# microsoft/Sora

Hardware: AMD Instinct MI355X
Metric: IQ Msamples/s through 802.11a 54 Mbps RX PHY (higher is better)
Workload: dtype int16 IQ / u8 path metrics

## Files before the change

sora_amd/build.py:

```python
import os
import shutil
import subprocess
import sys
from concurrent.futures import ThreadPoolExecutor

HERE = os.path.dirname(os.path.abspath(__file__))
CSRC = os.path.join(HERE, "csrc")
OBJ = os.path.join(HERE, "lib", "obj")
LIB = os.path.join(HERE, "lib", "libsora_hip.so")
SOURCES = ["k_scan.hip", "k_rx.hip", "k_vit16.hip", "k_vitwin.hip", "k_stage.hip", "k_tx.hip", "k_tx11n.hip", "k_tx_ht40.hip", "k_tx11b.hip", "k_mod.hip", "k_mod11n.hip", "k_mod11b.hip",
    "k_mod_ht40.hip", "k_11b.hip", "k_rx11b.hip", "k_11n.hip", "k_11a.hip", "k_rx11n.hip", "k_ht40.hip", "k_ht40_stages.hip", "k_deliver.hip", "sora_hip.cpp", "sora_shard.cpp"]
HEADERS = ["dev_arith.h", "dev_viterbi.h", "dev_vit16.h", "dev_winplan.h", "dev_vitwin.h", "dev_11n.h", "dev_ht40.h", "dev_pilot11a.h", "dev_sym11a.h", "dev_tx.h", "dev_11b.h", "dev_mod11b.h",
           "dev_cs11a.h", "rx_types.h", "kernels.h", "host_calls.h", "host_trellis.h", "host_stage.h", os.path.join("..", "..", "include", "sora_hip.h")]
FLAGS = ["--offload-arch=gfx950", "-O3", "-std=c++17", "-fPIC", "-fvisibility=hidden", "-x", "hip"]


def hipcc():
    for c in (os.environ.get("HIPCC"), shutil.which("hipcc"), "/opt/rocm/bin/hipcc"):
        if c and os.path.exists(c):
            return c
    raise RuntimeError("hipcc not found: libsora_hip.so cannot be built (there is no CPU fallback)")


def _newest_header():
    return max(os.path.getmtime(os.path.join(CSRC, h)) for h in HEADERS)


def _obj(src):
    return os.path.join(OBJ, os.path.splitext(src)[0] + ".o")


def _stale(src, hdr_t):
    o = _obj(src)
    return not os.path.exists(o) or os.path.getmtime(o) < max(os.path.getmtime(os.path.join(CSRC, src)), hdr_t)


def needs_build():
    if not os.path.exists(LIB):
        return True
    t = os.path.getmtime(LIB)
    return any(os.path.getmtime(os.path.join(CSRC, f)) > t for f in SOURCES + HEADERS)


INFO = os.path.join(HERE, "lib", "libsora_hip.buildinfo.json")


def sources_sha256():
    import hashlib
    h = hashlib.sha256()
    for f in sorted(SOURCES) + sorted(HEADERS):
        with open(os.path.join(CSRC, f), "rb") as fh:
            h.update(f.encode()); h.update(fh.read())
    return h.hexdigest()


def build_info():
    import json, socket, hashlib
    out = {"library": os.path.relpath(LIB, os.path.dirname(HERE)), "exists": os.path.exists(LIB)}
    if out["exists"]:
        with open(LIB, "rb") as fh:
            out["library_sha256"] = hashlib.sha256(fh.read()).hexdigest()
    try:
        with open(INFO) as fh:
            st = json.load(fh)
    except Exception:
        st = None
    now = sources_sha256()
    out["stamp"] = st
    out["sources_sha256_now"] = now
    out["built_from_this_tree"] = bool(st) and st.get("sources_sha256") == now and st.get("library_sha256") == out.get("library_sha256")
    out["built_on_this_host"] = bool(st) and st.get("host") == socket.gethostname()
    return out


def _write_info(ncompiled):
    import json, socket, hashlib, time
    try:
        ver = subprocess.run([hipcc(), "--version"], capture_output=True, text=True).stdout.splitlines()[0]
    except Exception:
        ver = None
    with open(LIB, "rb") as fh:
        lib_sha = hashlib.sha256(fh.read()).hexdigest()
    with open(INFO, "w") as fh:
        json.dump({"sources_sha256": sources_sha256(), "library_sha256": lib_sha, "host": socket.gethostname(), "built_at_unix": int(time.time()), "hipcc": ver,
                   "flags": FLAGS, "objects_compiled_in_this_build": ncompiled}, fh, indent=1)


def build_variant(name, defines):
    out_dir = os.path.join(HERE, "lib", "variants"); os.makedirs(out_dir, exist_ok=True)
    out = os.path.join(out_dir, name + ".so")
    if any(d.startswith(("SORA_DBG_", "SORA_SCAN_PROBE")) for d in defines) and "SORA_TOOLS" not in defines:
        defines = list(defines) + ["SORA_TOOLS"]
    cmd = [hipcc()] + FLAGS + ["-shared", "-w"] + ["-D" + d for d in defines] + [os.path.join(CSRC, f) for f in SOURCES] + ["-ldl", "-o", out]
    subprocess.check_call(cmd)
    return out


def build(force=False, verbose=False):
    if not force and not needs_build():
        return LIB
    os.makedirs(OBJ, exist_ok=True)
    cc = hipcc()
    hdr_t = _newest_header()
    todo = [s for s in SOURCES if force or _stale(s, hdr_t)]

    def compile_one(src):
        cmd = [cc] + FLAGS + ["-c", os.path.join(CSRC, src), "-o", _obj(src)]
        if verbose:
            print(" ".join(cmd))
        r = subprocess.run(cmd, capture_output=True, text=True)
        if r.returncode != 0:
            raise RuntimeError("hipcc failed on %s:\n%s" % (src, r.stderr[-4000:]))

    with ThreadPoolExecutor(max_workers=min(8, max(1, len(todo)))) as ex:
        list(ex.map(compile_one, todo))
    cmd = [cc, "--offload-arch=gfx950", "-shared", "-fPIC"] + [_obj(s) for s in SOURCES] + ["-ldl", "-o", LIB]
    if verbose:
        print(" ".join(cmd))
    subprocess.check_call(cmd)
    _write_info(len(todo))
    return LIB


if __name__ == "__main__":
    print(build(force="--force" in sys.argv, verbose=True))
```

sora_amd/csrc/dev_sym11a.h:

```cpp
#pragma once
#include "kernels.h"
#include "dev_viterbi.h"
#include "dev_pilot11a.h"

namespace sora {

__device__ __forceinline__ VitJob frame_vitjob(const FrameRow& r)
{
    VitJob J;
    J.valid = 1; J.soft_off = r.slot0 * (uint32_t)kSoftBytesPerSlot; J.nsoft = (uint32_t)r.nsym * 48u * r.nbpsc; J.length = r.length;
    J.dec_off = 0; J.out_off = r.slot0 * (uint32_t)kOutPerSlot; J.code_rate = r.code_rate; J.soft_bits = (uint32_t)kSoftScaled;
    return J;
}

static __device__ __constant__ PilotPolarity kPilotSgn = kPilotPolarity;
__device__ __forceinline__ int pilot_angle(int th, unsigned count) { return kPilotSgn.neg[count] ? w16(th + 0x8000) : th; }

template <typename COEF> __device__ __forceinline__ pcx sym_freq_comp(uint32_t raw, COEF fq) { return pk_cmul<15>(pk_sra(raw, 1), pk_tw_mul(fq)); }
template <typename COEF> __device__ __forceinline__ pcx sym_equalise(pcx y, COEF ch, int bin)
{
    return (bin >= 28 && bin < 36) ? 0u : pk_cmul<8>(y, pk_tw_mul(ch));
}
template <typename COEF>
__device__ __forceinline__ void sym_front_quad(const uint32_t raw[4], const COEF fq[4], const COEF ch[4], uint32_t* sl, int e, const Fft64TwPk& W, uint32_t o[4])
{
    pcx x[4];
#pragma unroll
    for (int m = 0; m < 4; m++) x[m] = sym_freq_comp(raw[m], fq[m]);
    fft64_core_pk(x, sl, e, W, wave_lds_sync);
    const unsigned rv = __brev((unsigned)e) >> 28;
#pragma unroll
    for (int q = 0; q < 4; q++) o[q] = sym_equalise(sl[rv + 16u * ((q & 1) * 2 + (q >> 1))], ch[q], 4 * e + q);
    wave_lds_sync();
}

constexpr int kSlotIters = 4;
constexpr uint32_t kNoOwner = 0xFFFFFFFFu;
struct WaveSlots {
    uint32_t first;
    uint32_t my_own;
    unsigned long long owned;
    uint32_t row0;
    bool one_frame;
    __device__ __forceinline__ uint32_t slot(int it, int g) const { return first + 4u * (uint32_t)it + (uint32_t)g; }
    __device__ __forceinline__ uint32_t owner(int it, int g) const { return (uint32_t)__shfl((int)my_own, 4 * it + g); }
    __device__ __forceinline__ unsigned quad(int it) const { return (unsigned)(owned >> (4 * it)) & 0xFu; }
};
__device__ __forceinline__ WaveSlots wave_slots(const RxArgs& A, uint32_t bid)
{
    const int w = threadIdx.x >> 6, lane = threadIdx.x & 63;
    WaveSlots S;
    S.first = (bid * 4u + (uint32_t)w) * (4u * kSlotIters);
    const uint32_t my_slot = S.first + (uint32_t)(lane & 15);
    S.my_own = (lane < 16 && my_slot < A.total_slots) ? A.slot_row[my_slot] : kNoOwner;
    S.owned = __ballot(S.my_own != kNoOwner);
    S.row0 = S.owned ? (uint32_t)__builtin_amdgcn_readlane((int)S.my_own, __builtin_ctzll(S.owned)) : kNoOwner;
    S.one_frame = __ballot(lane < 16 && S.my_own != kNoOwner && S.my_own != S.row0) == 0;
    return S;
}

__device__ __forceinline__ int4 track_advance(int th1, int th2, int th3, int th4, bool act, int& cfo_comp, int& sfo_comp, int& cfo_tr, int& sfo_tr)
{
    const int c0 = cfo_comp, s0 = sfo_comp;
    const int avg = w16((th1 + th2 + th3 + th4) / 4);
    const int del = w16(((th3 - th1) / 28 + (th4 - th2) / 28) >> 1);
    if (act) {
        cfo_tr = w16(cfo_tr + (avg >> 2)); sfo_tr = w16(sfo_tr + (del >> 2));
        cfo_comp = w16(cfo_comp + avg + cfo_tr); sfo_comp = w16(sfo_comp + del + sfo_tr);
    }
    return int4{ c0, s0, act ? avg : 0, act ? del : 0 };
}

__device__ __forceinline__ int4 track_rec4(TrackRec t) { return int4{ t.cfo_comp, t.sfo_comp, t.avg, t.del }; }
__device__ __forceinline__ void sym_back_demap(const Tables& T, const uint8_t* s_demap, const uint32_t v3[3], int4 rec, int nb, int e, uint8_t* dst)
{
    cpx c1[3], c2[3];
#pragma unroll
    for (int m = 0; m < 3; m++) {
        const int bin = carrier_bin48(e + 16 * m);
        const int c = bin < 32 ? bin : bin - 64;
        c1[m] = rot_coeff(T, w16(rec.x + c * rec.y));
        c2[m] = rot_coeff(T, w16(rec.z + c * rec.w));
    }
#pragma unroll
    for (int m = 0; m < 3; m++) {
        const int k = e + 16 * m;
        cpx v = mul_q15(unpack(v3[m]), c1[m]);
        v = mul_q15(v, c2[m]);
        int re = v.re >> 4, im = v.im >> 4;
        re = min(max(re, -128), 127); im = min(max(im, -128), 127);
        const unsigned ur = (unsigned)re & 0xFF, ui = (unsigned)im & 0xFF;
        uint8_t* o = dst + k * nb;
        const int h = nb >> 1;
        o[0] = s_demap[ur];
        if (nb >= 2) {
            o[h] = s_demap[ui];
            if (nb >= 4) {
                const int t1 = nb == 4 ? 256 : 512;
                o[1] = s_demap[t1 + ur]; o[h + 1] = s_demap[t1 + ui];
                if (nb == 6) { o[2] = s_demap[768 + ur]; o[5] = s_demap[768 + ui]; }
            }
        }
    }
}

__device__ __forceinline__ void demap_table_to_lds(const Tables& T, uint8_t* s_demap)
{
    reinterpret_cast<uint32_t*>(s_demap)[threadIdx.x] = (reinterpret_cast<const uint32_t*>(T.demap)[threadIdx.x] << 1) & 0xFEFEFEFEu;
}

__device__ __forceinline__ bool deint_packs(int nb, int lane) { return 8 * lane < 48 * nb; }
__device__ __forceinline__ void deint_map_words(const Tables& T, int nb, int lane, uint32_t mp[4])
{
    const uint16_t* map = T.deint + (nb == 1 ? 0 : nb == 2 ? 1 : nb == 4 ? 2 : 3) * 288;
    const bool packs = deint_packs(nb, lane);
#pragma unroll
    for (int t = 0; t < 4; t++) mp[t] = packs ? (uint32_t)map[8 * lane + 2 * t] | ((uint32_t)map[8 * lane + 2 * t + 1] << 16) : 0u;
}
__device__ __forceinline__ uint2 deint_gather8(const uint8_t* src, const uint32_t mp[4])
{
    uint32_t v[8];
#pragma unroll
    for (int t = 0; t < 4; t++) { v[2 * t] = src[mp[t] & 0xFFFFu]; v[2 * t + 1] = src[mp[t] >> 16]; }
    return uint2{ v[0] | (v[1] << 8) | (v[2] << 16) | (v[3] << 24), v[4] | (v[5] << 8) | (v[6] << 16) | (v[7] << 24) };
}
__device__ __forceinline__ void soft8_store(uint8_t* sym, uint32_t lane, uint2 b) { reinterpret_cast<uint2*>(sym)[lane] = b; }

}
```

sora_amd/csrc/k_rx.hip:

```cpp
#include <hip/hip_runtime.h>
#include <utility>
#include "kernels.h"
#include "dev_sym11a.h"
#include "dev_viterbi.h"
#include "dev_winplan.h"
#include "dev_vitwin.h"

namespace sora {

struct FrameLds {
    uint32_t eq[4][4][64];
    uint8_t  soft[4][4][288];
    uint8_t  demap[1024];
    int4     trk[4][4];
    int      nsym_of[4];
    short    st0[4][4];
};
template <bool SHARED>
__device__ __forceinline__ void frame_symbols(const RxArgs& A, uint32_t j, FrameLds& lds, bool valid = true)
{
    uint32_t (&s_eq)[4][4][64] = lds.eq; uint8_t (&s_soft)[4][4][288] = lds.soft; const uint8_t* s_demap = lds.demap;
    const int w = threadIdx.x >> 6, lane = threadIdx.x & 63, g = lane >> 4, e = lane & 15;
    const Tables& T = A.T;
    const uint32_t f = valid ? A.joblist[j] : 0u;
    FrameRow r = A.frames[f];
    if (!valid) { r.nsym = 0; r.nbpsc = 1; }
    if (lane == 0 && valid) A.jobs[j] = frame_vitjob(r);
    const FrameCtx* fx = A.fctx + f;
    const uint32_t* iq = A.iq + A.caps[r.capture].offset;
    const Fft64TwPk W = fft64_twiddles_pk(T, e);
    PkTw fq[4], ch[4];
#pragma unroll
    for (int m = 0; m < 4; m++) { fq[m] = pk_tw_mul(fx->freq[e + 16 * m]); ch[m] = pk_tw_mul(fx->chan[e + 16 * m]); }
    const int nb = __builtin_amdgcn_readfirstlane((int)r.nbpsc), ncbps = 48 * nb, nsym = __builtin_amdgcn_readfirstlane((int)r.nsym);
    uint32_t mp[4];
    const bool packs = deint_packs(nb, lane);
    deint_map_words(T, nb, lane, mp);
    uint8_t* dst = A.soft + (size_t)r.slot0 * kSoftBytesPerSlot;
    const int pk = lane & 3;
    const int pbin = pk == 0 ? 43 : pk == 1 ? 57 : pk == 2 ? 7 : 21, pc = pk == 0 ? -21 : pk == 1 ? -7 : pk == 2 ? 7 : 21;
    int cfo_comp = r.cfo_comp, sfo_comp = r.sfo_comp, cfo_tr = r.cfo_tracker, sfo_tr = r.sfo_tracker;
    unsigned symbol_count = 0;

    const uint32_t str_shift = A.str >> 1;
    auto load_samples = [&](int s0, uint32_t raw[4]) {
        const uint32_t p0 = r.data_start + __umul24(80u, (uint32_t)min(s0 + g, nsym)) + 8u + (uint32_t)e;
#pragma unroll
        for (int m = 0; m < 4; m++) raw[m] = iq[(p0 + 16u * (uint32_t)m) << str_shift];
    };
    int nsym_loop = nsym, nsym_f = nsym;
    if (SHARED) {
        if (lane == 0) { lds.nsym_of[w] = nsym; lds.st0[w][0] = (short)cfo_comp; lds.st0[w][1] = (short)sfo_comp; lds.st0[w][2] = (short)cfo_tr; lds.st0[w][3] = (short)sfo_tr; }
        __syncthreads();
        nsym_loop = max(max(lds.nsym_of[0], lds.nsym_of[1]), max(lds.nsym_of[2], lds.nsym_of[3]));
        const int fr = (lane >> 2) & 3;
        nsym_f = lds.nsym_of[fr];
        cfo_comp = lds.st0[fr][0]; sfo_comp = lds.st0[fr][1]; cfo_tr = lds.st0[fr][2]; sfo_tr = lds.st0[fr][3];
    }
    uint32_t raw[4] = { 0u, 0u, 0u, 0u };
    if (1 <= nsym) load_samples(1, raw);
    for (int s0 = 1; s0 <= nsym_loop; s0 += 4) {
        const int sym = s0 + g;
        const bool active = sym <= nsym;
        const bool mine = s0 <= nsym;
        int4 rec = { 0, 0, 0, 0 };
        if (mine) {
            pcx x[4], Y[4];
#pragma unroll
            for (int m = 0; m < 4; m++) x[m] = sym_freq_comp(raw[m], fq[m]);
            if (s0 + 4 <= nsym) load_samples(s0 + 4, raw);
            fft64_core_pk(x, s_eq[w][g], e, W, wave_lds_sync);
#pragma unroll
            for (int q = 0; q < 4; q++) Y[q] = s_eq[w][g][__brev((unsigned)(e + 16 * q)) >> 26];
            wave_lds_sync();
#pragma unroll
            for (int q = 0; q < 4; q++) s_eq[w][g][e + 16 * q] = sym_equalise(Y[q], ch[q], e + 16 * q);
            wave_lds_sync();
        }
        if (SHARED) {
            __syncthreads();
            if (w == 0) {
                const int fr = (lane >> 2) & 3;
#pragma unroll
                for (int gg = 0; gg < 4; gg++) {
                    const cpx p = mul_q15(unpack(s_eq[fr][gg][pbin]), rot_coeff(T, w16(cfo_comp + pc * sfo_comp)));
                    const int th = pilot_angle(pk == 3 ? uatan2(T, -p.im, -p.re) : uatan2(T, p.im, p.re), (symbol_count + (unsigned)gg) % 127u);
                    int th1 = __builtin_amdgcn_update_dpp(0, th, 0x00, 0xF, 0xF, true), th2 = __builtin_amdgcn_update_dpp(0, th, 0x55, 0xF, 0xF, true);
                    int th3 = __builtin_amdgcn_update_dpp(0, th, 0xAA, 0xF, 0xF, true), th4 = __builtin_amdgcn_update_dpp(0, th, 0xFF, 0xF, 0xF, true);
                    asm volatile("" : "+v"(th1), "+v"(th2), "+v"(th3), "+v"(th4));
                    const int4 t = track_advance(th1, th2, th3, th4, s0 + gg <= nsym_f, cfo_comp, sfo_comp, cfo_tr, sfo_tr);
                    if (lane < 16 && pk == 0) lds.trk[fr][gg] = t;
                }
            }
            symbol_count = (symbol_count + 4u) % 127u;
            __syncthreads();
            rec = lds.trk[w][g];
        } else {
            int4 t[4];
#pragma unroll
            for (int gg = 0; gg < 4; gg++) {
                t[gg] = int4{ cfo_comp, sfo_comp, 0, 0 };
                if (s0 + gg <= nsym) {
                    const cpx p = mul_q15(unpack(s_eq[w][gg][pbin]), rot_coeff(T, w16(cfo_comp + pc * sfo_comp)));
                    const int th = pilot_angle(pk == 3 ? uatan2(T, -p.im, -p.re) : uatan2(T, p.im, p.re), symbol_count);
                    symbol_count++; if (symbol_count >= 127) symbol_count = 0;
                    t[gg] = track_advance(__builtin_amdgcn_readlane(th, 0), __builtin_amdgcn_readlane(th, 1), __builtin_amdgcn_readlane(th, 2), __builtin_amdgcn_readlane(th, 3),
                                          true, cfo_comp, sfo_comp, cfo_tr, sfo_tr);
                }
            }
            rec = t[0];
            if (g == 1) rec = t[1]; else if (g == 2) rec = t[2]; else if (g == 3) rec = t[3];
        }
        if (!mine) continue;
        if (active) {
            uint32_t v3[3];
#pragma unroll
            for (int m = 0; m < 3; m++) v3[m] = s_eq[w][g][carrier_bin48(e + 16 * m)];
            sym_back_demap(T, s_demap, v3, rec, nb, e, s_soft[w][g]);
        }
        wave_lds_sync();
        {
            const int nact = min(4, nsym - s0 + 1);
            const uint32_t sym_bytes = (uint32_t)ncbps;
            uint8_t* d = dst + (size_t)(s0 - 1) * sym_bytes;
            for (int gs = 0; gs < nact; gs++, d += sym_bytes)
                if (packs) soft8_store(d, (uint32_t)lane, deint_gather8(s_soft[w][gs], mp));
        }
        wave_lds_sync();
    }
}
__global__ void __launch_bounds__(256) k_frame(RxArgs A)
{
    __shared__ FrameLds lds;
    demap_table_to_lds(A.T, lds.demap);
    __syncthreads();
    if (!locate_job(blockIdx.x * 4, A.njobs).ok) return;
    const JobRef jr = locate_job(blockIdx.x * 4 + (threadIdx.x >> 6), A.njobs);
    frame_symbols<true>(A, jr.ok ? jr.list * A.nrows + jr.idx : 0u, lds, jr.ok);
}

typedef uint32_t u32x4_t __attribute__((ext_vector_type(4)));
__device__ __forceinline__ void store16_through(uint4* p, uint4 v)
{
    const u32x4_t x = { v.x, v.y, v.z, v.w };
    asm volatile("global_store_dwordx4 %0, %1, off sc1\n\ts_nop 1" : : "v"(p), "v"(x) : "memory");
}
__device__ __forceinline__ void store4_through(uint32_t* p, uint32_t v) { __hip_atomic_store(p, v, __ATOMIC_RELAXED, __HIP_MEMORY_SCOPE_AGENT); }

template <bool THROUGH>
__device__ __forceinline__ void sym_front_block(const RxArgs& A, uint32_t bid, uint32_t (*s_eq)[4][64])
{
    const int w = threadIdx.x >> 6, lane = threadIdx.x & 63, g = lane >> 4, e = lane & 15;
    const Tables& T = A.T;
    const WaveSlots S = wave_slots(A, bid);
    if (S.owned == 0) return;
    uint32_t own[kSlotIters];
#pragma unroll
    for (int it = 0; it < kSlotIters; it++) own[it] = S.owner(it, g);
    const Fft64TwPk W = fft64_twiddles_pk(T, e);
    uint32_t* sl = s_eq[w][g];
    uint4* eq4 = reinterpret_cast<uint4*>(A.eq);
    auto store = [&](uint32_t slot, const uint32_t o[4]) {
        if (THROUGH) store16_through(eq4 + ((size_t)slot * 16u + (uint32_t)e), uint4{ o[0], o[1], o[2], o[3] });
        else eq4[(size_t)slot * 16u + (uint32_t)e] = uint4{ o[0], o[1], o[2], o[3] };
        auto pilot = [&](uint32_t k, uint32_t v) { if (THROUGH) store4_through(A.pil + ((size_t)slot * 4u + k), v); else A.pil[(size_t)slot * 4u + k] = v; };
        if (e == 10) pilot(0u, o[3]);
        if (e == 14) pilot(1u, o[1]);
        if (e == 1)  pilot(2u, o[3]);
        if (e == 5)  pilot(3u, o[1]);
    };
    if (S.one_frame) {
        const FrameRow& r = A.frames[S.row0];
        const uint32_t* iq = A.iq + A.caps[r.capture].offset;
        const uint32_t ds = r.data_start, s0 = r.slot0, str = A.str;
        const FrameCtx* fx = A.fctx + S.row0;
        uint32_t raw[kSlotIters][4];
#pragma unroll
        for (int it = 0; it < kSlotIters; it++) {
            const uint32_t p0 = ds + 80u * (S.slot(it, g) - s0) + 8u;
#pragma unroll
            for (int m = 0; m < 4; m++) raw[it][m] = own[it] != kNoOwner ? iq[(size_t)(p0 + (uint32_t)(e + 16 * m)) * str] : 0u;
        }
        PkTw fq[4], ch[4];
#pragma unroll
        for (int m = 0; m < 4; m++) { fq[m] = pk_tw_mul(fx->freq[e + 16 * m]); ch[m] = pk_tw_mul(fx->chan[4 * e + m]); }
#pragma unroll
        for (int it = 0; it < kSlotIters; it++) {
            if (S.quad(it) == 0) continue;
            uint32_t o[4];
            sym_front_quad(raw[it], fq, ch, sl, e, W, o);
            if (own[it] != kNoOwner) store(S.slot(it, g), o);
        }
        return;
    }
#pragma unroll 1
    for (int it = 0; it < kSlotIters; it++) {
        if (S.quad(it) == 0) continue;
        const uint32_t ow = S.owner(it, g);
        const bool mine = ow != kNoOwner;
        const uint32_t slot = S.slot(it, g);
        uint32_t raw[4] = { 0u, 0u, 0u, 0u };
        PkTw fq[4], ch[4];
        const FrameCtx* fx = A.fctx + (mine ? ow : 0u);
        if (mine) {
            const FrameRow& r = A.frames[ow];
            const uint32_t* iq = A.iq + A.caps[r.capture].offset;
            const uint32_t p0 = r.data_start + 80u * (slot - r.slot0) + 8u;
#pragma unroll
            for (int m = 0; m < 4; m++) raw[m] = iq[(size_t)(p0 + (uint32_t)(e + 16 * m)) * A.str];
        }
#pragma unroll
        for (int m = 0; m < 4; m++) { fq[m] = pk_tw_mul(mine ? fx->freq[e + 16 * m] : 0u); ch[m] = pk_tw_mul(mine ? fx->chan[4 * e + m] : 0u); }
        uint32_t o[4];
        sym_front_quad(raw, fq, ch, sl, e, W, o);
        if (mine) store(slot, o);
    }
}

__global__ void __launch_bounds__(256) k_sym_front(RxArgs A)
{
    __shared__ uint32_t s_eq[4][4][64];
    sym_front_block<false>(A, blockIdx.x, s_eq);
}

__device__ __forceinline__ uint2 track_step(const TrkTables& s_t, uint32_t cur, int flip, int pc, int m3, int& cfo, int& sfo, int& ctr, int& str)
{
    constexpr float kInv28 = 0.0357142873108387f;
    const unsigned a = (unsigned)(cfo + pc * sfo) & 0xFFFFu;
    const int qi = trk_quarter_index(a);
    const int sraw = s_t.q[qi], craw = s_t.q[16384 - qi];
    const uint32_t ws = s_t.e2s[a >> 4], wc = s_t.e2c[a >> 4];
    const int ms = __builtin_amdgcn_sbfe((int)a, 15, 1), mc = __builtin_amdgcn_sbfe((int)(a ^ (a << 1)), 15, 1);
    const int sn = ((sraw ^ ms) - ms) + trk_sext2(ws, a), cs = ((craw ^ mc) - mc) + trk_sext2(wc, a);
    const int pr = (int)(short)cur, pi = (int)cur >> 16;
    const int re = __builtin_amdgcn_sbfe(pr * cs + pi * sn, 15, 16), im = __builtin_amdgcn_sbfe(pi * cs - pr * sn, 15, 16);
    const int x = (re ^ m3) - m3, y = (im ^ m3) - m3;
    const int sh = max(25 - __builtin_clz((unsigned)(max(x, -x) | max(y, -y)) | 1u), 0);
    int th = trk_uatan2_entry(s_t, y >> sh, x >> sh);
    th = __builtin_amdgcn_sbfe(th ^ flip, 0, 16);
    int th1, th2, th3, th4;
    asm volatile("s_nop 1\n\t"
                 "v_mov_b32_dpp %0, %4 quad_perm:[0,0,0,0] row_mask:0xf bank_mask:0xf bound_ctrl:1\n\t"
                 "v_mov_b32_dpp %1, %4 quad_perm:[1,1,1,1] row_mask:0xf bank_mask:0xf bound_ctrl:1\n\t"
                 "v_mov_b32_dpp %2, %4 quad_perm:[2,2,2,2] row_mask:0xf bank_mask:0xf bound_ctrl:1\n\t"
                 "v_mov_b32_dpp %3, %4 quad_perm:[3,3,3,3] row_mask:0xf bank_mask:0xf bound_ctrl:1"
                 : "=&v"(th1), "=&v"(th2), "=&v"(th3), "=&v"(th4) : "v"(th));
    const int sum = th1 + th2 + th3 + th4;
    const int avg = (sum + ((sum >> 31) & 3)) >> 2;
    const int del = ((int)((float)(th3 - th1) * kInv28) + (int)((float)(th4 - th2) * kInv28)) >> 1;
    const uint2 rec = uint2{ __builtin_amdgcn_perm((uint32_t)sfo, (uint32_t)cfo, 0x05040100u), __builtin_amdgcn_perm((uint32_t)del, (uint32_t)avg, 0x05040100u) };
    ctr += avg >> 2; str += del >> 2;
    cfo = (int)((unsigned)cfo + (unsigned)avg + (unsigned)ctr); sfo = __builtin_amdgcn_sbfe(sfo + del + str, 0, 16);
    return rec;
}

__device__ __forceinline__ void track_tables_to_lds(const uint32_t* __restrict__ trk, TrkTables& s_t, uint32_t* s_pol)
{
    if (threadIdx.x < 127) {
        unsigned b = 0;
#pragma unroll
        for (unsigned u = 0; u < 8; u++) b |= pilot_sgn((threadIdx.x + u) % 127u) << u;
        s_pol[threadIdx.x] = b;
    }
    const uint4* src = reinterpret_cast<const uint4*>(trk);
    uint4* dst = reinterpret_cast<uint4*>(&s_t);
    constexpr uint32_t kWords = sizeof(TrkTables) / 16, kBatch = 11;
    for (uint32_t i0 = threadIdx.x; i0 < kWords; i0 += 256u * kBatch) {
        uint4 v[kBatch];
#pragma unroll
        for (uint32_t b = 0; b < kBatch; b++) v[b] = src[min(i0 + 256u * b, kWords - 1u)];
#pragma unroll
        for (uint32_t b = 0; b < kBatch; b++) if (i0 + 256u * b < kWords) dst[i0 + 256u * b] = v[b];
    }
}

__global__ void __launch_bounds__(256) k_track_lds(RxArgs A)
{
    __shared__ TrkTables s_t;
    __shared__ uint32_t s_pol[128];
    track_tables_to_lds(A.T.trk, s_t, s_pol);
    __syncthreads();
    const int lane = threadIdx.x & 63, pk = lane & 3;
    const JobRef jr = locate_job(blockIdx.x * 64u + (threadIdx.x >> 2), A.njobs);
    const uint32_t j = jr.ok ? jr.list * A.nrows + jr.idx : 0u;
    const uint32_t f = jr.ok ? A.joblist[j] : 0u;
    const FrameRow r = A.frames[f];
    const int nsym = jr.ok ? (int)r.nsym : 0;
    if (jr.ok && pk == 0) A.jobs[j] = frame_vitjob(r);
    const int pc = pk == 0 ? -21 : pk == 1 ? -7 : pk == 2 ? 7 : 21;
    const int m3 = pk == 3 ? -1 : 0;
    int cfo = r.cfo_comp, sfo = r.sfo_comp, ctr = r.cfo_tracker, str = r.sfo_tracker;
    int nmax = nsym;
#pragma unroll
    for (int o = 32; o >= 4; o >>= 1) nmax = max(nmax, __shfl_xor(nmax, o));
    nmax = __builtin_amdgcn_readfirstlane(nmax);
    const uint32_t w0 = (jr.ok ? (r.slot0 + 1u) * 4u + (uint32_t)pk : (uint32_t)pk) * 4u;
    const uint32_t t0 = (jr.ok ? r.slot0 + 1u : A.total_slots + 1u) * 8u;
    const char* __restrict__ pil = reinterpret_cast<const char*>(A.pil);
    char* __restrict__ trk2 = reinterpret_cast<char*>(A.track);
    const unsigned last = (unsigned)max(nsym, 1) - 1u, nrec = (unsigned)nsym;
    constexpr int kAhead = 8;
    uint32_t q[kAhead];
#pragma unroll
    for (int i = 0; i < kAhead; i++) q[i] = *reinterpret_cast<const uint32_t*>(pil + (w0 + 16u * min((unsigned)i, last)));
    unsigned cnt = 0;
    for (int s0 = 1; s0 <= nmax; s0 += kAhead) {
        const unsigned pol = (unsigned)__builtin_amdgcn_readfirstlane((int)s_pol[cnt]);
        cnt = cnt + (unsigned)kAhead >= 127u ? cnt + (unsigned)kAhead - 127u : cnt + (unsigned)kAhead;
#pragma unroll
        for (int u = 0; u < kAhead; u++) {
            const int s = s0 + u;
            const uint32_t cur = q[u];
            q[u] = *reinterpret_cast<const uint32_t*>(pil + (w0 + 16u * min((unsigned)(s + kAhead - 1), last)));
            const int flip = (int)((pol << (15 - u)) & 0x8000u);
            *reinterpret_cast<uint2*>(trk2 + (t0 + 8u * min((unsigned)(s - 1), nrec))) = track_step(s_t, cur, flip, pc, m3, cfo, sfo, ctr, str);
        }
    }
}

__global__ void __launch_bounds__(256) k_sym_back(RxArgs A)
{
    __shared__ uint8_t s_soft[4][4][288];
    __shared__ uint8_t s_demap[1024];
    const int w = threadIdx.x >> 6, lane = threadIdx.x & 63, g = lane >> 4, e = lane & 15;
    const Tables& T = A.T;
    demap_table_to_lds(T, s_demap);
    __syncthreads();
    const WaveSlots S = wave_slots(A, blockIdx.x);
    if (S.owned == 0) return;
    int bins[3];
#pragma unroll
    for (int m = 0; m < 3; m++) bins[m] = carrier_bin48(e + 16 * m);
    if (S.one_frame) {
        const FrameRow& r = A.frames[S.row0];
        const int nb = __builtin_amdgcn_readfirstlane((int)r.nbpsc), ncbps = 48 * nb;
        const uint32_t slot0 = (uint32_t)__builtin_amdgcn_readfirstlane((int)r.slot0), sym_bytes = (uint32_t)ncbps;
        uint8_t* stream = A.soft + (size_t)slot0 * kSoftBytesPerSlot;
        const bool packs = deint_packs(nb, lane);
        uint32_t mp[4];
        deint_map_words(T, nb, lane, mp);
        TrackRec tr[kSlotIters]; uint32_t v3[kSlotIters][3];
#pragma unroll
        for (int it = 0; it < kSlotIters; it++) {
            const uint32_t slot = S.slot(it, g);
            const bool mine = (S.quad(it) >> g) & 1u;
            tr[it] = mine ? A.track[slot] : TrackRec{ 0, 0, 0, 0 };
#pragma unroll
            for (int m = 0; m < 3; m++) v3[it][m] = mine ? A.eq[(size_t)slot * 64u + (uint32_t)bins[m]] : 0u;
        }
#pragma unroll
        for (int it = 0; it < kSlotIters; it++) {
            const unsigned quad = S.quad(it);
            if (quad == 0) continue;
            if ((quad >> g) & 1u) sym_back_demap(T, s_demap, v3[it], track_rec4(tr[it]), nb, e, s_soft[w][g]);
            wave_lds_sync();
#pragma unroll
            for (int gs = 0; gs < 4; gs++) {
                if (!((quad >> gs) & 1u) || !packs) continue;
                const uint32_t sg = S.slot(it, gs);
                soft8_store(stream + (size_t)(sg - slot0 - 1u) * sym_bytes, (uint32_t)lane, deint_gather8(s_soft[w][gs], mp));
            }
            wave_lds_sync();
        }
        return;
    }
    int cur_nb = 0; uint32_t mp[4] = { 0, 0, 0, 0 };
#pragma unroll 1
    for (int it = 0; it < kSlotIters; it++) {
        const unsigned quad = S.quad(it);
        if (quad == 0) continue;
        const uint32_t ow = S.owner(it, g);
        const bool mine = ow != kNoOwner;
        const uint32_t slot = S.slot(it, g);
        int nb = 0; uint32_t slot0 = 0;
        if (mine) {
            const FrameRow& r = A.frames[ow];
            nb = r.nbpsc; slot0 = r.slot0;
            uint32_t v3[3];
#pragma unroll
            for (int m = 0; m < 3; m++) v3[m] = A.eq[(size_t)slot * 64u + (uint32_t)bins[m]];
            sym_back_demap(T, s_demap, v3, track_rec4(A.track[slot]), nb, e, s_soft[w][g]);
        }
        wave_lds_sync();
#pragma unroll 1
        for (int gs = 0; gs < 4; gs++) {
            if (!((quad >> gs) & 1u)) continue;
            const int nbg = __shfl(nb, 16 * gs);
            const uint32_t slot0g = (uint32_t)__shfl((int)slot0, 16 * gs);
            if (nbg != cur_nb) { cur_nb = nbg; deint_map_words(T, nbg, lane, mp); }
            if (deint_packs(nbg, lane)) {
                const uint32_t sg = S.slot(it, gs);
                uint8_t* d = A.soft + (size_t)slot0g * kSoftBytesPerSlot + (size_t)(sg - slot0g - 1u) * (48u * (uint32_t)nbg);
                soft8_store(d, (uint32_t)lane, deint_gather8(s_soft[w][gs], mp));
            }
        }
        wave_lds_sync();
    }
}

constexpr uint32_t kPipeMaxSym = 1376;
constexpr uint32_t kPipeRing = 512;
struct PipeTrackLds {
    TrkTables t;
    uint32_t pol[128];
    uint32_t pil[kPipeMaxSym][4];
    uint2 rec[kPipeRing];
    uint8_t demap[1024];
    uint8_t soft[3][4][288];
    uint32_t done;
    uint32_t next_quad[3];
    uint32_t give_up;
    uint32_t pad[11];
};
constexpr uint32_t kPipeLdsBytes = sizeof(PipeTrackLds);
static_assert(kPipeLdsBytes <= 160 * 1024 && sizeof(TrkTables) % 16 == 0, "k_pipe: a tracker workgroup's LDS");
static_assert(4 * sizeof(Lds16<256, 24>) <= kPipeLdsBytes, "k_pipe: four trellis waves' LDS");

#ifdef SORA_DBG_PIPE_TIMELINE
#define PIPE_STAMP(P, i) do { if ((threadIdx.x & 63) == 0) (P).flags[(P).stamp_base + (i)] = (uint32_t)wall_clock64(); } while (0)
#else
#define PIPE_STAMP(P, i) do {} while (0)
#endif
__device__ __forceinline__ uint32_t flag_load(const uint32_t* p) { return __hip_atomic_load(p, __ATOMIC_RELAXED, __HIP_MEMORY_SCOPE_AGENT); }
__device__ __forceinline__ bool pipe_expired(long long t0, uint32_t wait_ticks) { return wall_clock64() - t0 > (long long)wait_ticks; }

__device__ __forceinline__ void pipe_track_block(const RxArgs& A, const PipeArgs& P, uint32_t t, PipeTrackLds& L)
{
    const int w = threadIdx.x >> 6, lane = threadIdx.x & 63;
    const JobRef jr = locate_job(t, A.njobs);
// ... 539 lines not shown
```

Baseline: 55660.

## Write demapped soft bits directly in deinterleaved column order to drop gather

Each lane now demaps carriers 3e..3e+2 and scatters the soft bytes straight into their deinterleaved positions in LDS, using per-lane precomputed table offsets that fold the 802.11a second-permutation rotation into the demap table choice. The store stage then reads contiguous 8-byte words instead of running an indexed 8-byte gather through a deinterleave map. This removes the gather and map setup but relies on the column formulas exactly matching the standard interleaver, and adds scattered byte writes to LDS.

Result: no change. 55800, median of 2 (+0.3%).

```diff
diff --git a/sora_amd/build.py b/sora_amd/build.py
--- a/sora_amd/build.py
+++ b/sora_amd/build.py
@@ -10,8 +10,8 @@
 LIB = os.path.join(HERE, "lib", "libsora_hip.so")
 SOURCES = ["k_scan.hip", "k_rx.hip", "k_vit16.hip", "k_vitwin.hip", "k_stage.hip", "k_tx.hip", "k_tx11n.hip", "k_tx_ht40.hip", "k_tx11b.hip", "k_mod.hip", "k_mod11n.hip", "k_mod11b.hip",
     "k_mod_ht40.hip", "k_11b.hip", "k_rx11b.hip", "k_11n.hip", "k_11a.hip", "k_rx11n.hip", "k_ht40.hip", "k_ht40_stages.hip", "k_deliver.hip", "sora_hip.cpp", "sora_shard.cpp"]
-HEADERS = ["dev_arith.h", "dev_viterbi.h", "dev_vit16.h", "dev_winplan.h", "dev_vitwin.h", "dev_11n.h", "dev_ht40.h", "dev_pilot11a.h", "dev_sym11a.h", "dev_tx.h", "dev_11b.h", "dev_mod11b.h",
-           "dev_cs11a.h", "rx_types.h", "kernels.h", "host_calls.h", "host_trellis.h", "host_stage.h", os.path.join("..", "..", "include", "sora_hip.h")]
+HEADERS = ["dev_arith.h", "dev_viterbi.h", "dev_vit16.h", "dev_winplan.h", "dev_vitwin.h", "dev_11n.h", "dev_ht40.h", "dev_pilot11a.h", "dev_sym11a.h", "deint_columns.h", "dev_tx.h", "dev_11b.h",
+           "dev_mod11b.h", "dev_cs11a.h", "rx_types.h", "kernels.h", "host_calls.h", "host_trellis.h", "host_stage.h", os.path.join("..", "..", "include", "sora_hip.h")]
 FLAGS = ["--offload-arch=gfx950", "-O3", "-std=c++17", "-fPIC", "-fvisibility=hidden", "-x", "hip"]
 
 
diff --git a/sora_amd/csrc/deint_columns.h b/sora_amd/csrc/deint_columns.h
--- /dev/null
+++ b/sora_amd/csrc/deint_columns.h
@@ -0,0 +1,10 @@
+#pragma once
+
+namespace sora {
+
+constexpr int deint_group(int nb) { return nb >= 2 ? nb / 2 : 1; }
+constexpr int deint_column_row(int nb, int r, int u) { return deint_group(nb) * (u / deint_group(nb)) + (u % deint_group(nb) + r) % deint_group(nb); }
+constexpr int deint_column_depth(int nb, int r, int t) { return (t + deint_group(nb) - r % deint_group(nb)) % deint_group(nb); }
+constexpr int deint_column_byte(int nb, int r, int u) { return 16 * deint_column_row(nb, r, u) + r; }
+
+}
diff --git a/sora_amd/csrc/dev_sym11a.h b/sora_amd/csrc/dev_sym11a.h
--- a/sora_amd/csrc/dev_sym11a.h
+++ b/sora_amd/csrc/dev_sym11a.h
@@ -2,6 +2,7 @@
 #include "kernels.h"
 #include "dev_viterbi.h"
 #include "dev_pilot11a.h"
+#include "deint_columns.h"
 
 namespace sora {
 
@@ -104,6 +105,49 @@
     }
 }
 
+__device__ __forceinline__ void demap_column_tables(int nb, int e, int tb[3])
+{
+#pragma unroll
+    for (int t = 0; t < 3; t++) {
+        const int d = nb < 4 ? 0 : nb == 4 ? deint_column_depth(4, e, t & 1) : deint_column_depth(6, e, t);
+        tb[t] = d == 0 ? 0 : d == 1 ? (nb == 4 ? 256 : 512) : 768;
+    }
+}
+__device__ __forceinline__ void sym_back_demap_stream(const Tables& T, const uint8_t* s_demap, const int tb[3], const uint32_t v3[3], int4 rec, int nb, int e, uint8_t* row)
+{
+    cpx c1[3], c2[3];
+#pragma unroll
+    for (int m = 0; m < 3; m++) {
+        const int bin = carrier_bin48(3 * e + m);
+        const int c = bin < 32 ? bin : bin - 64;
+        c1[m] = rot_coeff(T, w16(rec.x + c * rec.y));
+        c2[m] = rot_coeff(T, w16(rec.z + c * rec.w));
+    }
+    const int h = nb >> 1;
+#pragma unroll
+    for (int m = 0; m < 3; m++) {
+        cpx v = mul_q15(unpack(v3[m]), c1[m]);
+        v = mul_q15(v, c2[m]);
+        int re = v.re >> 4, im = v.im >> 4;
+        re = min(max(re, -128), 127); im = min(max(im, -128), 127);
+        uint8_t* o = row + 16 * nb * m;
+        const uint8_t r0 = s_demap[tb[0] | (re & 0xFF)];
+        if (nb >= 2) {
+            const uint8_t i0 = s_demap[tb[0] | (im & 0xFF)];
+            if (nb >= 4) {
+                const uint8_t r1 = s_demap[tb[1] | (re & 0xFF)], i1 = s_demap[tb[1] | (im & 0xFF)];
+                if (nb == 6) {
+                    const uint8_t r2 = s_demap[tb[2] | (re & 0xFF)], i2 = s_demap[tb[2] | (im & 0xFF)];
+                    o[32] = r2; o[80] = i2;
+                }
+                o[16] = r1; o[16 * (h + 1)] = i1;
+            }
+            o[16 * h] = i0;
+        }
+        o[0] = r0;
+    }
+}
+
 __device__ __forceinline__ void demap_table_to_lds(const Tables& T, uint8_t* s_demap)
 {
     reinterpret_cast<uint32_t*>(s_demap)[threadIdx.x] = (reinterpret_cast<const uint32_t*>(T.demap)[threadIdx.x] << 1) & 0xFEFEFEFEu;
diff --git a/sora_amd/csrc/k_rx.hip b/sora_amd/csrc/k_rx.hip
--- a/sora_amd/csrc/k_rx.hip
+++ b/sora_amd/csrc/k_rx.hip
@@ -33,9 +33,9 @@
 #pragma unroll
     for (int m = 0; m < 4; m++) { fq[m] = pk_tw_mul(fx->freq[e + 16 * m]); ch[m] = pk_tw_mul(fx->chan[e + 16 * m]); }
     const int nb = __builtin_amdgcn_readfirstlane((int)r.nbpsc), ncbps = 48 * nb, nsym = __builtin_amdgcn_readfirstlane((int)r.nsym);
-    uint32_t mp[4];
     const bool packs = deint_packs(nb, lane);
-    deint_map_words(T, nb, lane, mp);
+    int tb[3];
+    demap_column_tables(nb, e, tb);
     uint8_t* dst = A.soft + (size_t)r.slot0 * kSoftBytesPerSlot;
     const int pk = lane & 3;
     const int pbin = pk == 0 ? 43 : pk == 1 ? 57 : pk == 2 ? 7 : 21, pc = pk == 0 ? -21 : pk == 1 ? -7 : pk == 2 ? 7 : 21;
@@ -115,8 +115,8 @@
         if (active) {
             uint32_t v3[3];
 #pragma unroll
-            for (int m = 0; m < 3; m++) v3[m] = s_eq[w][g][carrier_bin48(e + 16 * m)];
-            sym_back_demap(T, s_demap, v3, rec, nb, e, s_soft[w][g]);
+            for (int m = 0; m < 3; m++) v3[m] = s_eq[w][g][carrier_bin48(3 * e + m)];
+            sym_back_demap_stream(T, s_demap, tb, v3, rec, nb, e, s_soft[w][g] + e);
         }
         wave_lds_sync();
         {
@@ -124,7 +124,7 @@
             const uint32_t sym_bytes = (uint32_t)ncbps;
             uint8_t* d = dst + (size_t)(s0 - 1) * sym_bytes;
             for (int gs = 0; gs < nact; gs++, d += sym_bytes)
-                if (packs) soft8_store(d, (uint32_t)lane, deint_gather8(s_soft[w][gs], mp));
+                if (packs) soft8_store(d, (uint32_t)lane, reinterpret_cast<const uint2*>(s_soft[w][gs])[lane]);
         }
         wave_lds_sync();
     }
```
